# Quantum-Chemistry-Group-BNU/PyNQS

Measured on AMD Instinct MI355X. Metric: local energies/sec (whole node), higher is better.
Workload: dtype f64

## Files before the change

pynqs_amd/csrc/kernels_rbm_forward.hip:

```cpp
#include "detcore.h"
#include "launch.h"
#include "rbm_math.h"

namespace pynqs {

constexpr int kHChunk = 8;

struct Prod {
  double re = 1.0, im = 0.0;
  double lin = 0.0, ang = 0.0;
  int e2 = 0;
  __device__ __forceinline__ void renorm() {
    int k;
    (void)frexp(fmax(fabs(re), fabs(im)), &k);
    re = ldexp(re, -k); im = ldexp(im, -k);
    e2 += k;
  }
  __device__ __forceinline__ bool finite() const { return fabs(re) < __builtin_inf() && fabs(im) < __builtin_inf(); }
  template <bool CPLX>
  __device__ __forceinline__ void times_2cosh(double x, double y) {
    const double ax = fabs(x);
    const double rho = exp(-2.0 * ax);
    lin += ax;
    if constexpr (CPLX) {
      const double sy = x < 0.0 ? -y : y;
      double sn, cs;
      sincos_mod(-2.0 * sy, sn, cs);
      const double u = fma(rho, cs, 1.0), v = rho * sn;
      const double nr = re * u - im * v;
      im = fma(re, v, im * u);
      re = nr;
      ang += sy;
    } else {
      re *= 1.0 + rho;
    }
  }
};

template <int FLAVOUR>
__device__ __forceinline__ void write_psi(double *__restrict__ psi, int64_t i, const Prod &P, double axr, double axi) {
  const double kLn2 = 0.693147180559945309417;
  if constexpr (FLAVOUR == PYNQS_RBM_REAL) {
    psi[i] = P.re * exp(axr + P.lin + kLn2 * (double)P.e2);
  } else if constexpr (FLAVOUR == PYNQS_RBM_TANH) {
    psi[i] = tanh(axr) * P.re * exp(P.lin + kLn2 * (double)P.e2);
  } else if constexpr (FLAVOUR == PYNQS_RBM_PHASE) {
    double sn, cs;
    sincos(axr + P.lin + log(P.re) + kLn2 * (double)P.e2, &sn, &cs);
    psi[2 * i] = cs; psi[2 * i + 1] = sn;
  } else {
    const double m = exp(axr + P.lin + kLn2 * (double)P.e2);
    double sn, cs;
    sincos(axi + P.ang, &sn, &cs);
    psi[2 * i] = m * (P.re * cs - P.im * sn);
    psi[2 * i + 1] = m * (P.re * sn + P.im * cs);
  }
}

template <int LEN, int FLAVOUR>
__device__ __forceinline__ void rbm_forward_row(const uint64_t (&ket)[LEN], int sorb, int H, const double *__restrict__ W,
                                                const double *__restrict__ hb, const double *__restrict__ vb, Prod &P, double &axr, double &axi) {
  constexpr bool CPLX = FLAVOUR == PYNQS_RBM_COMPLEX;
  for (int h0 = 0; h0 < H; h0 += kHChunk) {
    double tr[kHChunk], ti[kHChunk];
#pragma unroll
    for (int j = 0; j < kHChunk; ++j) {
      const int h = min(h0 + j, H - 1);
      tr[j] = CPLX ? hb[2 * h] : hb[h];
      ti[j] = CPLX ? hb[2 * h + 1] : 0.0;
    }
    for (int o = 0; o < sorb; ++o) {
      const double x = pm1_of<LEN>(ket, o);
#pragma unroll
      for (int j = 0; j < kHChunk; ++j) {
        const int h = min(h0 + j, H - 1);
        if constexpr (CPLX) {
          tr[j] = fma(x, W[((size_t)h * sorb + o) * 2], tr[j]);
          ti[j] = fma(x, W[((size_t)h * sorb + o) * 2 + 1], ti[j]);
        } else {
          tr[j] = fma(x, W[(size_t)h * sorb + o], tr[j]);
        }
      }
    }
#pragma unroll
    for (int j = 0; j < kHChunk; ++j)
      if (h0 + j < H) P.template times_2cosh<CPLX>(tr[j], ti[j]);
    P.renorm();
  }
  axr = 0.0; axi = 0.0;
  if (vb) {
    for (int o = 0; o < sorb; ++o) {
      const double x = pm1_of<LEN>(ket, o);
      if constexpr (CPLX) { axr = fma(x, vb[2 * o], axr); axi = fma(x, vb[2 * o + 1], axi); }
      else axr = fma(x, vb[o], axr);
    }
  }
}

template <int LEN, int FLAVOUR>
__global__ __launch_bounds__(kBlock) void rbm_forward_kernel(const uint64_t *__restrict__ onv, int64_t n, int sorb, int H,
                                                             const double *__restrict__ W, const double *__restrict__ hb,
                                                             const double *__restrict__ vb, double *__restrict__ psi) {
  const int64_t i = (int64_t)blockIdx.x * kBlock + threadIdx.x;
  const int64_t row = i < n ? i : n - 1;
  uint64_t ket[LEN];
#pragma unroll
  for (int w = 0; w < LEN; ++w) ket[w] = onv[row * LEN + w];
  Prod P;
  double axr, axi;
  rbm_forward_row<LEN, FLAVOUR>(ket, sorb, H, W, hb, vb, P, axr, axi);
  if (i >= n) return;
  write_psi<FLAVOUR>(psi, i, P, axr, axi);
}

__host__ __device__ inline int children_hp(int H) { return (H + 2) | 1; }

template <bool CPLX>
__global__ __launch_bounds__(kBlock) void rbm_children_factors_kernel(int sorb, int H, const double *__restrict__ W, const double *__restrict__ vb,
                                                                      double *__restrict__ factors) {
  constexpr int C = CPLX ? 2 : 1;
  const int HP = children_hp(H);
  const int idx = blockIdx.x * kBlock + threadIdx.x;
  if (idx == 0) factors[(size_t)(2 * sorb + 1) * HP * C] = 0.0;
  if (idx >= (2 * sorb + 1) * HP) return;
  const int row = idx / HP, h = idx - row * HP, o = row >> 1;
  const double sign = (row & 1) ? -1.0 : 1.0;
  double re = 0.0, im = 0.0;
  if (row == 2 * sorb) {
    re = h < H ? 1.0 : 0.0;
  } else if (h < H) {
    const double wr = W[((size_t)h * sorb + o) * C], wi = CPLX ? W[((size_t)h * sorb + o) * C + 1] : 0.0;
    const double m = fabs(4.0 * wr) <= 80.0 ? exp(-4.0 * sign * wr) : __builtin_nan("");
    if constexpr (CPLX) {
      double sn, cs;
      sincos(-4.0 * sign * wi, &sn, &cs);
      re = m * cs; im = m * sn;
    } else {
      re = m;
    }
  } else if (h == H) {
#pragma unroll 16
    for (int k = 0; k < H; ++k) {
      re += W[((size_t)k * sorb + o) * C];
      if constexpr (CPLX) im += W[((size_t)k * sorb + o) * C + 1];
    }
    re *= 2.0 * sign; im *= 2.0 * sign;
  } else if (h == H + 1 && vb) {
    re = 2.0 * sign * vb[(size_t)o * C];
    if constexpr (CPLX) im = 2.0 * sign * vb[(size_t)o * C + 1];
  }
  factors[(size_t)idx * C] = re;
  if constexpr (CPLX) factors[(size_t)idx * C + 1] = im;
}

constexpr int kParentChunk = 4;

template <int LEN, bool CPLX>
__global__ __launch_bounds__(kBlock) void rbm_children_parents_kernel(const uint64_t *__restrict__ onv, int64_t n, int sorb, int H,
                                                                      const double *__restrict__ W, const double *__restrict__ hb,
                                                                      const double *__restrict__ vb, const double *__restrict__ factors,
                                                                      double *__restrict__ table) {
  constexpr int C = CPLX ? 2 : 1;
  const int64_t i = (int64_t)blockIdx.x * kBlock + threadIdx.x;
  const int64_t row = i < n ? i : n - 1;
  const int h0 = (int)blockIdx.y * kParentChunk;
  uint64_t ket[LEN];
#pragma unroll
  for (int w = 0; w < LEN; ++w) ket[w] = onv[row * LEN + w];
  double *__restrict__ out = table + (size_t)row * (size_t)(H + 2) * C;
  double tr[kParentChunk], ti[kParentChunk];
#pragma unroll
  for (int j = 0; j < kParentChunk; ++j) {
    const int h = min(h0 + j, H - 1);
    tr[j] = CPLX ? hb[2 * h] : hb[h];
    ti[j] = CPLX ? hb[2 * h + 1] : 0.0;
  }
  for (int o = 0; o < sorb; ++o) {
    const double x = pm1_of<LEN>(ket, o);
#pragma unroll
    for (int j = 0; j < kParentChunk; ++j) {
      const int h = min(h0 + j, H - 1);
      tr[j] = fma(x, W[((size_t)h * sorb + o) * C], tr[j]);
      if constexpr (CPLX) ti[j] = fma(x, W[((size_t)h * sorb + o) * C + 1], ti[j]);
    }
  }
#pragma unroll
  for (int j = 0; j < kParentChunk; ++j) {
    if (h0 + j < H && i < n) {
      if (!(tr[j] > -340.0)) const_cast<double *>(factors)[(size_t)(2 * sorb + 1) * children_hp(H) * C] = 1.0;
      const double m = exp(-2.0 * tr[j]);
      if constexpr (CPLX) {
        double sn, cs;
        sincos_mod(-2.0 * ti[j], sn, cs);
        out[(size_t)(h0 + j) * 2] = m * cs;
        out[(size_t)(h0 + j) * 2 + 1] = m * sn;
      } else {
        out[h0 + j] = m;
      }
    }
  }
  if (blockIdx.y != 0) return;
  const int HP = children_hp(H);
  double sr = 0.0, si = 0.0, axr = 0.0, axi = 0.0;
  for (int h = 0; h < H; ++h) {
    sr += hb[(size_t)h * C];
    if constexpr (CPLX) si += hb[(size_t)h * C + 1];
  }
  for (int o = 0; o < sorb; ++o) {
    const double x = pm1_of<LEN>(ket, o);
    const double *__restrict__ f = factors + ((size_t)(2 * o) * HP + H) * C;
    sr = fma(0.5 * x, f[0], sr);
    axr = fma(0.5 * x, f[C], axr);
    if constexpr (CPLX) { si = fma(0.5 * x, f[1], si); axi = fma(0.5 * x, f[C + 1], axi); }
  }
  if (i >= n) return;
  out[(size_t)H * C] = sr;
  out[(size_t)(H + 1) * C] = axr;
  if constexpr (CPLX) { out[(size_t)H * C + 1] = si; out[(size_t)(H + 1) * C + 1] = axi; }
}

#ifndef PYNQS_CHILD_BLOCK
#define PYNQS_CHILD_BLOCK 1024
#endif
constexpr int kChildBlock = PYNQS_CHILD_BLOCK;

template <int LEN, int FLAVOUR>
__global__ __launch_bounds__(kChildBlock) void rbm_forward_children_kernel(const uint64_t *__restrict__ onv, int64_t n, const int32_t *__restrict__ count_dev,
                                                                      const int32_t *__restrict__ parent, const uint64_t *__restrict__ walkers,
                                                                      int64_t nwalkers, const double *__restrict__ table,
                                                                      const double *__restrict__ factors, int sorb, int H,
                                                                      const double *__restrict__ W, const double *__restrict__ hb,
                                                                      const double *__restrict__ vb, double *__restrict__ psi) {
  constexpr bool CPLX = FLAVOUR == PYNQS_RBM_COMPLEX;
  constexpr int C = CPLX ? 2 : 1;
  extern __shared__ __attribute__((aligned(16))) double wl[];
  const int HP = children_hp(H);
  int64_t cnt = n;
  if (count_dev) cnt = min((int64_t)max(*count_dev, 0), n);
  if (factors[(size_t)(2 * sorb + 1) * HP * C] != 0.0) {
    const int64_t rounds = (cnt + (int64_t)gridDim.x * kChildBlock - 1) / ((int64_t)gridDim.x * kChildBlock);
    for (int64_t r = 0; r < rounds; ++r) {
      const int64_t i = ((int64_t)r * gridDim.x + blockIdx.x) * kChildBlock + threadIdx.x;
      const int64_t row = i < cnt ? i : cnt - 1;
      uint64_t ket[LEN];
#pragma unroll
      for (int w = 0; w < LEN; ++w) ket[w] = onv[row * LEN + w];
      Prod P;
      double axr, axi;
      rbm_forward_row<LEN, FLAVOUR>(ket, sorb, H, W, hb, vb, P, axr, axi);
      if (i < cnt) write_psi<FLAVOUR>(psi, i, P, axr, axi);
    }
    return;
  }
  for (int idx = threadIdx.x; idx < (2 * sorb + 1) * HP * C; idx += kChildBlock) wl[idx] = factors[idx];
  __syncthreads();
  for (int64_t i = (int64_t)blockIdx.x * kChildBlock + threadIdx.x; i < cnt; i += (int64_t)gridDim.x * kChildBlock) {
    int64_t p = parent[i];
    bool stranger = p < 0 || p >= nwalkers;
    p = stranger ? 0 : p;
    int at[4];
#pragma unroll
    for (int q = 0; q < 4; ++q) at[q] = 2 * sorb * HP;
    int k = 0, nflip = 0;
#pragma unroll
    for (int w = 0; w < LEN; ++w) {
      const uint64_t xc = onv[i * LEN + w];
      uint64_t d = xc ^ walkers[p * LEN + w];
      nflip += __popcll(d);
#pragma unroll
      for (int t = 0; t < 4; ++t) {
        if (d && k < 4) {
          const int b = __builtin_ctzll(d);
          d &= d - 1;
          const int r = (2 * (64 * w + b) + (((xc >> b) & 1ull) ? 0 : 1)) * HP;
#pragma unroll
          for (int q = 0; q < 4; ++q)
            if (q == k) at[q] = r;
          ++k;
        }
      }
    }
    const double *__restrict__ tp = table + (size_t)p * (size_t)(H + 2) * C;
    Prod P;
    for (int h0 = 0; h0 < H; h0 += kHChunk) {
#pragma unroll
      for (int j = 0; j < kHChunk; ++j) {
        const int h = h0 + j;
        if (h < H) {
          double qr = tp[(size_t)h * C], qi = CPLX ? tp[(size_t)h * C + 1] : 0.0;
#pragma unroll
          for (int q = 0; q < 4; ++q) {
            const double fr = wl[(size_t)(at[q] + h) * C];
            if constexpr (CPLX) {
              const double fi = wl[(size_t)(at[q] + h) * C + 1];
              const double nr = qr * fr - qi * fi;
              qi = fma(qr, fi, qi * fr);
              qr = nr;
            } else {
              qr *= fr;
            }
          }
          if constexpr (CPLX) {
            const double u = 1.0 + qr;
            const double nr = P.re * u - P.im * qi;
            P.im = fma(P.re, qi, P.im * u);
            P.re = nr;
          } else {
            P.re *= 1.0 + qr;
          }
        }
      }
      P.renorm();
    }
    double axr = tp[(size_t)(H + 1) * C], axi = CPLX ? tp[(size_t)(H + 1) * C + 1] : 0.0;
    P.lin = tp[(size_t)H * C];
    P.ang = CPLX ? tp[(size_t)H * C + 1] : 0.0;
#pragma unroll
    for (int q = 0; q < 4; ++q) {
      P.lin += wl[(size_t)(at[q] + H) * C];
      axr += wl[(size_t)(at[q] + H + 1) * C];
      if constexpr (CPLX) {
        P.ang += wl[(size_t)(at[q] + H) * C + 1];
        axi += wl[(size_t)(at[q] + H + 1) * C + 1];
      }
    }
    stranger = stranger || nflip > 4 || !P.finite();
    if (__ballot(stranger)) {
      uint64_t ket[LEN];
#pragma unroll
      for (int w = 0; w < LEN; ++w) ket[w] = onv[i * LEN + w];
      Prod P2;
      double a2r, a2i;
      rbm_forward_row<LEN, FLAVOUR>(ket, sorb, H, W, hb, vb, P2, a2r, a2i);
      if (stranger) { P = P2; axr = a2r; axi = a2i; }
    }
    write_psi<FLAVOUR>(psi, i, P, axr, axi);
  }
}

template <int LEN, int FLAVOUR>
__global__ __launch_bounds__(kBlock) void rbm_forward_children_wave_kernel(const uint64_t *__restrict__ onv, int64_t n, const int32_t *__restrict__ count_dev,
                                                                           const int32_t *__restrict__ parent, const uint64_t *__restrict__ walkers,
                                                                           int64_t nwalkers, const double *__restrict__ table,
                                                                           const double *__restrict__ factors, int sorb, int H,
                                                                           const double *__restrict__ W, const double *__restrict__ hb,
                                                                           const double *__restrict__ vb, double *__restrict__ psi) {
  constexpr bool CPLX = FLAVOUR == PYNQS_RBM_COMPLEX;
  constexpr int C = CPLX ? 2 : 1;
  const int HP = children_hp(H);
  int64_t cnt = n;
  if (count_dev) cnt = min((int64_t)max(*count_dev, 0), n);
  if (factors[(size_t)(2 * sorb + 1) * HP * C] != 0.0) {
    const int64_t rounds = (cnt + (int64_t)gridDim.x * kBlock - 1) / ((int64_t)gridDim.x * kBlock);
    for (int64_t r = 0; r < rounds; ++r) {
      const int64_t i = ((int64_t)r * gridDim.x + blockIdx.x) * kBlock + threadIdx.x;
      const int64_t row = i < cnt ? i : cnt - 1;
      uint64_t ket[LEN];
#pragma unroll
      for (int w = 0; w < LEN; ++w) ket[w] = onv[row * LEN + w];
      Prod P;
      double axr, axi;
      rbm_forward_row<LEN, FLAVOUR>(ket, sorb, H, W, hb, vb, P, axr, axi);
      if (i < cnt) write_psi<FLAVOUR>(psi, i, P, axr, axi);
    }
    return;
  }
  const int lane = threadIdx.x & 63;
  const int wave = __builtin_amdgcn_readfirstlane((int)(threadIdx.x >> 6));
  const int64_t nwaves = (int64_t)gridDim.x * (kBlock / 64);
  constexpr int kWaveRows = 16;
  for (int64_t i0 = ((int64_t)blockIdx.x * (kBlock / 64) + wave) * kWaveRows; i0 < cnt; i0 += nwaves * kWaveRows)
  for (int64_t i = i0; i < min(i0 + kWaveRows, cnt); ++i) {
    int64_t p = parent[i];
    bool stranger = p < 0 || p >= nwalkers;
    p = stranger ? 0 : p;
    int at[4];
#pragma unroll
    for (int q = 0; q < 4; ++q) at[q] = 2 * sorb * HP;
    int k = 0, nflip = 0;
#pragma unroll
    for (int w = 0; w < LEN; ++w) {
      const uint64_t xc = onv[i * LEN + w];
      uint64_t d = xc ^ walkers[p * LEN + w];
      nflip += __popcll(d);
#pragma unroll
      for (int t = 0; t < 4; ++t) {
        if (d && k < 4) {
          const int b = __builtin_ctzll(d);
          d &= d - 1;
          const int r = (2 * (64 * w + b) + (((xc >> b) & 1ull) ? 0 : 1)) * HP;
#pragma unroll
          for (int q = 0; q < 4; ++q)
            if (q == k) at[q] = r;
          ++k;
        }
      }
    }
    const auto from_scratch = [&]() {
      uint64_t ket[LEN];
#pragma unroll
      for (int w = 0; w < LEN; ++w) ket[w] = onv[i * LEN + w];
      Prod P2;
      double a2r, a2i;
      rbm_forward_row<LEN, FLAVOUR>(ket, sorb, H, W, hb, vb, P2, a2r, a2i);
      if (lane == 0) write_psi<FLAVOUR>(psi, i, P2, a2r, a2i);
    };
    if (stranger || nflip > 4) {
      from_scratch();
      continue;
    }
    const double *__restrict__ tp = table + (size_t)p * (size_t)(H + 2) * C;
    Prod P;
    for (int h = lane; h < H; h += 64) {
      double qr = tp[(size_t)h * C], qi = CPLX ? tp[(size_t)h * C + 1] : 0.0;
#pragma unroll
      for (int q = 0; q < 4; ++q) {
        const double fr = factors[(size_t)(at[q] + h) * C];
        if constexpr (CPLX) {
          const double fi = factors[(size_t)(at[q] + h) * C + 1];
          const double nr = qr * fr - qi * fi;
          qi = fma(qr, fi, qi * fr);
          qr = nr;
        } else {
          qr *= fr;
        }
      }
      if constexpr (CPLX) {
        const double u = 1.0 + qr;
        const double nr = P.re * u - P.im * qi;
        P.im = fma(P.re, qi, P.im * u);
        P.re = nr;
      } else {
        P.re *= 1.0 + qr;
      }
      P.renorm();
    }
#pragma unroll
    for (int d = 32; d > 0; d >>= 1) {
      const double orr = __shfl_xor(P.re, d), oi = CPLX ? __shfl_xor(P.im, d) : 0.0;
      const int oe = __shfl_xor(P.e2, d);
      if constexpr (CPLX) {
        const double nr = P.re * orr - P.im * oi;
        P.im = fma(P.re, oi, P.im * orr);
        P.re = nr;
      } else {
        P.re *= orr;
      }
      P.e2 += oe;
    }
    P.renorm();
    if (__ballot(!P.finite())) {
      from_scratch();
      continue;
    }
    if (lane == 0) {
      double axr = tp[(size_t)(H + 1) * C], axi = CPLX ? tp[(size_t)(H + 1) * C + 1] : 0.0;
      P.lin = tp[(size_t)H * C];
      P.ang = CPLX ? tp[(size_t)H * C + 1] : 0.0;
#pragma unroll
      for (int q = 0; q < 4; ++q) {
        P.lin += factors[(size_t)(at[q] + H) * C];
        axr += factors[(size_t)(at[q] + H + 1) * C];
        if constexpr (CPLX) {
          P.ang += factors[(size_t)(at[q] + H) * C + 1];
          axi += factors[(size_t)(at[q] + H + 1) * C + 1];
        }
      }
      write_psi<FLAVOUR>(psi, i, P, axr, axi);
    }
  }
}

}

using namespace pynqs;

extern "C" int pynqs_rbm_forward(const uint64_t *onv, int64_t n, int sorb, const double *weights, const double *hidden_bias,
                                 const double *visible_bias, int nhidden, int flavour, double *psi, void *stream) {
  pynqs::DeviceScope device_scope_(onv);
  if (n < 0 || n > 0x7fffffffll * kBlock || sorb < 1 || sorb > kMaxSorb || nhidden < 1) return set_error(PYNQS_EINVAL, "bad n/sorb/nhidden");
  if (flavour != PYNQS_RBM_REAL && flavour != PYNQS_RBM_TANH && flavour != PYNQS_RBM_PHASE && flavour != PYNQS_RBM_COMPLEX)
    return set_error(PYNQS_EINVAL, "bad flavour");
  if (n == 0) return PYNQS_OK;
  if (!onv || !weights || !hidden_bias || !psi) return set_error(PYNQS_EINVAL, "null pointer");
  const int len = (sorb - 1) / 64 + 1;
  const uint32_t grid = (uint32_t)((n + kBlock - 1) / kBlock);
  hipStream_t st = (hipStream_t)stream;
#define PYNQS_RF(F) hipLaunchKernelGGL((rbm_forward_kernel<LEN, F>), dim3(grid), dim3(kBlock), 0, st, onv, n, sorb, nhidden, weights, hidden_bias, visible_bias, psi)
  DISPATCH_LEN(len, {
    switch (flavour) {
      case PYNQS_RBM_REAL: PYNQS_RF(PYNQS_RBM_REAL); break;
      case PYNQS_RBM_TANH: PYNQS_RF(PYNQS_RBM_TANH); break;
      case PYNQS_RBM_PHASE: PYNQS_RF(PYNQS_RBM_PHASE); break;
      default: PYNQS_RF(PYNQS_RBM_COMPLEX); break;
    }
  });
#undef PYNQS_RF
  return check_launch("rbm_forward");
}

static size_t children_lds_bytes(int sorb, int nhidden, int flavour) {
  return (size_t)(2 * sorb + 1) * (size_t)children_hp(nhidden) * (flavour == PYNQS_RBM_COMPLEX ? 16 : 8);
}

static bool children_flavour_ok(int flavour) {
  return flavour == PYNQS_RBM_REAL || flavour == PYNQS_RBM_TANH || flavour == PYNQS_RBM_PHASE || flavour == PYNQS_RBM_COMPLEX;
}

extern "C" int pynqs_rbm_forward_children_supported(int sorb, int nhidden, int flavour) {
  if (sorb < 1 || sorb > kMaxSorb || nhidden < 1 || !children_flavour_ok(flavour)) return 0;
  return 1;
}
static bool children_table_in_lds(int sorb, int nhidden, int flavour) {
  static const int force = getenv("PYNQS_RBM_CHILDREN_WAVE") ? atoi(getenv("PYNQS_RBM_CHILDREN_WAVE")) : -1;
  return force != 1 && children_lds_bytes(sorb, nhidden, flavour) <= 64 * 1024;
}

extern "C" int64_t pynqs_rbm_children_table_bytes(int64_t nwalkers, int sorb, int nhidden, int flavour) {
  if (nwalkers < 0 || sorb < 1 || sorb > kMaxSorb || nhidden < 1 || !children_flavour_ok(flavour)) return -1;
  const int64_t c = flavour == PYNQS_RBM_COMPLEX ? 16 : 8;
  return nwalkers * (nhidden + 2) * c + (int64_t)children_lds_bytes(sorb, nhidden, flavour) + 8;
}

extern "C" int pynqs_rbm_children_prepare(const uint64_t *walkers, int64_t nwalkers, int sorb, const double *weights, const double *hidden_bias,
                                          const double *visible_bias, int nhidden, int flavour, void *table, void *stream) {
  pynqs::DeviceScope device_scope_(table);
  if (nwalkers < 0 || nwalkers > 0x7fffffffll * kBlock || sorb < 1 || sorb > kMaxSorb || nhidden < 1 || !children_flavour_ok(flavour))
    return set_error(PYNQS_EINVAL, "bad nwalkers/sorb/nhidden/flavour");
  if (!weights || !hidden_bias || !table || (nwalkers > 0 && !walkers)) return set_error(PYNQS_EINVAL, "null pointer");
  const bool cplx = flavour == PYNQS_RBM_COMPLEX;
  const int len = (sorb - 1) / 64 + 1;
  hipStream_t st = (hipStream_t)stream;
  double *parents = (double *)table;
  double *factors = parents + (size_t)nwalkers * (size_t)(nhidden + 2) * (cplx ? 2 : 1);
  const uint32_t gf = (uint32_t)(((2 * sorb + 1) * children_hp(nhidden) + kBlock - 1) / kBlock);
  if (cplx) hipLaunchKernelGGL((rbm_children_factors_kernel<true>), dim3(gf), dim3(kBlock), 0, st, sorb, nhidden, weights, visible_bias, factors);
  else hipLaunchKernelGGL((rbm_children_factors_kernel<false>), dim3(gf), dim3(kBlock), 0, st, sorb, nhidden, weights, visible_bias, factors);
  if (nwalkers > 0) {
    const dim3 grid((uint32_t)((nwalkers + kBlock - 1) / kBlock), (uint32_t)((nhidden + kParentChunk - 1) / kParentChunk));
    if (grid.y > 65535u) return set_error(PYNQS_EINVAL, "too many hidden units");
    DISPATCH_LEN(len, {
      if (cplx)
        hipLaunchKernelGGL((rbm_children_parents_kernel<LEN, true>), grid, dim3(kBlock), 0, st, walkers, nwalkers, sorb, nhidden, weights,
                           hidden_bias, visible_bias, factors, parents);
      else
        hipLaunchKernelGGL((rbm_children_parents_kernel<LEN, false>), grid, dim3(kBlock), 0, st, walkers, nwalkers, sorb, nhidden, weights,
                           hidden_bias, visible_bias, factors, parents);
    });
  }
  return check_launch("rbm_children_prepare");
}

extern "C" int pynqs_rbm_forward_children(const uint64_t *onv, int64_t n, const int32_t *count_dev, const int32_t *parent,
                                          const uint64_t *walkers, int64_t nwalkers, const void *table, int sorb, const double *weights,
                                          const double *hidden_bias, const double *visible_bias, int nhidden, int flavour, double *psi,
                                          void *stream) {
  pynqs::DeviceScope device_scope_(onv);
  if (n < 0 || n > 0x7fffffffll * kBlock || nwalkers < 0 || sorb < 1 || sorb > kMaxSorb || nhidden < 1) return set_error(PYNQS_EINVAL, "bad n/sorb/nhidden");
  if (!pynqs_rbm_forward_children_supported(sorb, nhidden, flavour))
    return set_error(PYNQS_EINVAL, "rbm_forward_children: bad flavour");
  if (n == 0) return PYNQS_OK;
  if (!onv || !parent || !walkers || !table || !psi || !weights || !hidden_bias || nwalkers == 0) return set_error(PYNQS_EINVAL, "null pointer");
  const int len = (sorb - 1) / 64 + 1;
  int64_t blocks = (n + kChildBlock - 1) / kChildBlock;
  if (blocks > 1024) blocks = 1024;
  const uint32_t grid = (uint32_t)blocks;
  const size_t lds = children_lds_bytes(sorb, nhidden, flavour);
  const double *parents = (const double *)table;
  const double *factors = parents + (size_t)nwalkers * (size_t)(nhidden + 2) * (flavour == PYNQS_RBM_COMPLEX ? 2 : 1);
  hipStream_t st = (hipStream_t)stream;
  const bool in_lds = children_table_in_lds(sorb, nhidden, flavour);
  int64_t wblocks = (n + (kBlock / 64) * 16 - 1) / ((kBlock / 64) * 16);
  if (wblocks > 256 * 32) wblocks = 256 * 32;
#define PYNQS_RC(F)                                                                                                                          \
  do {                                                                                                                                       \
    if (in_lds)                                                                                                                              \
      hipLaunchKernelGGL((rbm_forward_children_kernel<LEN, F>), dim3(grid), dim3(kChildBlock), lds, st, onv, n, count_dev, parent, walkers,  \
                         nwalkers, parents, factors, sorb, nhidden, weights, hidden_bias, visible_bias, psi);                                \
    else                                                                                                                                     \
      hipLaunchKernelGGL((rbm_forward_children_wave_kernel<LEN, F>), dim3((uint32_t)wblocks), dim3(kBlock), 0, st, onv, n, count_dev,        \
                         parent, walkers, nwalkers, parents, factors, sorb, nhidden, weights, hidden_bias, visible_bias, psi);               \
  } while (0)
  DISPATCH_LEN(len, {
    switch (flavour) {
      case PYNQS_RBM_REAL: PYNQS_RC(PYNQS_RBM_REAL); break;
      case PYNQS_RBM_TANH: PYNQS_RC(PYNQS_RBM_TANH); break;
      case PYNQS_RBM_PHASE: PYNQS_RC(PYNQS_RBM_PHASE); break;
      default: PYNQS_RC(PYNQS_RBM_COMPLEX); break;
    }
  });
#undef PYNQS_RC
  return check_launch("rbm_forward_children");
}
```

pynqs_amd/csrc/kernels_reduce_onepass.hip:

```cpp
#include "detcore.h"
#include "launch.h"
#include "plan.h"
#include "plan_dev.h"
#include "plan_tiles.h"
#include "reduce_common.h"
#include "reduce_list.h"

namespace pynqs {




template <int LEN, typename T, bool SAMPLED>
struct KeepSink {
  T eps;
  uint32_t chunk, nchunks, tS;
  int64_t seg_base;
  volatile uint32_t *run;
  WinnerList wl;
  uint32_t *bufc;
  T *bufh;
  volatile uint32_t *dstat;
  double *tsum;
  uint32_t *kept_total;
// ... 303 lines not shown
__global__ __launch_bounds__(kBlock) void reduce_onepass_kernel(const uint64_t *__restrict__ bra, SDParams p, PlanLayout pl, uint32_t nchunks,
                                                                uint32_t chunk_len, uint32_t max_tiles, const T *__restrict__ plan, T eps,
                                                                uint32_t nsample, uint64_t seed, uint32_t wl_cap, OnepassOut<T> o) {
  extern __shared__ __attribute__((aligned(16))) unsigned char smem[];
  __shared__ uint32_t next_tile, kept_total, wl_n;
  __shared__ int32_t wl_base;
  __shared__ uint32_t wave_run[kBlock / 64];
  __shared__ double s_part[kBlock / 64 + 1];
  __shared__ uint32_t s_parti[kBlock / 64 + 1];
  uint64_t walker;
  uint32_t chunk;
  map_workgroup(nchunks, false, walker, chunk);
  o.parent = (int32_t)walker;
  const uint64_t slot = walker * nchunks + chunk;
  const int tid = threadIdx.x, lane = tid & 63, wave = tid >> 6;
  const int64_t seg_base = (int64_t)slot * ((int64_t)o.fixed + o.cap_d);
  if (tid == 0) { next_tile = 0; kept_total = 0; wl_n = 0; }
  unsigned char *extra = smem + ((lds_bytes(p, sizeof(T)) + 15) & ~(size_t)15);
  volatile uint32_t *dstat = reinterpret_cast<volatile uint32_t *>(extra);
  extra += ((size_t)max_tiles * 4 + 15) & ~(size_t)15;
  double *tsum = reinterpret_cast<double *>(extra);
  uint32_t *dinfo = reinterpret_cast<uint32_t *>(extra + (SAMPLED ? (size_t)max_tiles * 8 : 0));
  WinnerList wl;
  wl.n = &wl_n;
  wl.cap = wl_cap;
  wl.slot = reinterpret_cast<uint32_t *>(smem + onepass_lds(p, sizeof(T), max_tiles, SAMPLED, 0));
  wl.col = wl.slot + wl_cap;
  for (uint32_t i = tid; i < max_tiles; i += kBlock) {
    dstat[i] = 0u;
    if constexpr (SAMPLED) { tsum[i] = 0.0; dinfo[i] = 0u; }
  }
  for (uint32_t i = tid; i < o.fixed; i += kBlock) o.rec_col[seg_base + i] = -1;
  if constexpr (SAMPLED) {
    for (uint32_t i = tid; i < nsample; i += kBlock) o.srec_col[(int64_t)walker * nsample + i] = -1;
  }
  Walker<LEN> wk;
  load_walker<LEN>(bra + walker * LEN, wk);
  const LdsLayout L = carve_lds(smem, p);
  const int nocc = build_walker_tables<LEN>(wk, p, L);

  const uint32_t tS_all = (p.d1 + kSinglesPerTile - 1) / kSinglesPerTile;
  const uint32_t tS = tS_all > chunk ? (tS_all - chunk + nchunks - 1) / nchunks : 0;
  T *quarter = reinterpret_cast<T *>(L.scratch) + wave * (kDiagTile / 4);
  {
    KeepSink<LEN, T, SAMPLED> sink;
    sink.eps = eps; sink.chunk = chunk; sink.nchunks = nchunks; sink.tS = tS; sink.seg_base = seg_base;
    sink.run = wave_run + wave; sink.wl = wl;
    sink.bufh = quarter;
    sink.bufc = reinterpret_cast<uint32_t *>(quarter + kOneTileCols);
    sink.dstat = dstat; sink.tsum = tsum; sink.kept_total = &kept_total;
    sink.p = &p; sink.L = &L; sink.wk = &wk; sink.o = o; sink.tile = 0xffffffffu; sink.sub = 0.0;
    visit_tiles<LEN, T>(p, pl, L, nocc, plan, wk, nchunks, chunk, chunk_len, 0u, &next_tile, sink);
    sink.flush();
  }
  flush_winner_list<LEN, T>(o, wl, &wl_base, p, L, wk);
  if (tid == 0) {
    o.seg_count[slot] = (int32_t)kept_total;
    if (kept_total > o.cap_d) {
      atomicOr(reinterpret_cast<unsigned int *>(o.counters + 1), 1u);
      atomicMax(o.counters + 2, (int32_t)kept_total);
    }
  }
  if constexpr (SAMPLED) {
    const uint32_t per = (max_tiles + kBlock - 1) / kBlock;
    const uint32_t b0 = min((uint32_t)tid * per, max_tiles), b1 = min(b0 + per, max_tiles);
    double local = 0.0;
    for (uint32_t i = b0; i < b1; ++i) local += tsum[i];
    double incl = op_scan(local, lane);
    if (lane == 63) s_part[wave] = incl;
    __syncthreads();
    double before = 0.0, total = 0.0;
    for (int w = 0; w < kBlock / 64; ++w) {
      if (w < wave) before += s_part[w];
      total += s_part[w];
    }
    double run = before + incl - local;
    for (uint32_t i = b0; i < b1; ++i) { run += tsum[i]; tsum[i] = run; }
    __syncthreads();
    const double Srow = total;
    if (tid == 0 && o.row_sum) o.row_sum[walker] = Srow;
    const uint64_t key = op_mix64((o.seed_dev ? seed + *o.seed_dev : seed) ^ op_mix64(slot));
    if (Srow > 0.0) {
      for (uint32_t k = tid; k < nsample; k += kBlock) {
        const uint64_t r = op_mix64(key ^ op_mix64(0xffffffff00000000ull | k));
        const double target = (double)(r >> 11) * 0x1.0p-53 * Srow;
        uint32_t lo = 0, hi = max_tiles;
        while (lo < hi) {
          const uint32_t mid = (lo + hi) >> 1;
          if (tsum[mid] > target) hi = mid; else lo = mid + 1;
        }
        if (lo >= max_tiles) lo = max_tiles - 1;
        while (lo > 0 && !(tsum[lo] > tsum[lo - 1])) --lo;
        atomicAdd(&dinfo[lo], 1u);
      }
    }
    __syncthreads();
    uint32_t lsum = 0;
    for (uint32_t i = b0; i < b1; ++i) lsum += dinfo[i];
    uint32_t iscan = lsum;
#pragma unroll
    for (int d = 1; d < 64; d <<= 1) {
      const uint32_t ov = __shfl_up(iscan, d);
      if (lane >= d) iscan += ov;
    }
    if (lane == 63) s_parti[wave] = iscan;
    __syncthreads();
    uint32_t ibefore = 0;
    for (int w = 0; w < wave; ++w) ibefore += s_parti[w];
    uint32_t off = ibefore + iscan - lsum;
    for (uint32_t i = b0; i < b1; ++i) {
      const uint32_t c = dinfo[i];
      dinfo[i] = (off << 16) | c;
      off += c;
    }
    if (tid == 0) next_tile = 0;
    __syncthreads();
    unsigned char *mine = reinterpret_cast<unsigned char *>(dinfo) + (((size_t)max_tiles * 4 + 15) & ~(size_t)15) + (size_t)wave * kDrawLdsPerWave;
    DrawLds S;
    S.prefix = reinterpret_cast<double *>(mine);
    S.run = reinterpret_cast<volatile double *>(mine + (size_t)kOneTileCols * 8);
    S.cs = reinterpret_cast<uint32_t *>(mine + (size_t)kOneTileCols * 8 + 8);
    S.hits = S.cs + kOneTileCols;
    S.ncols = reinterpret_cast<volatile uint32_t *>(S.hits + kOneTileCols);
    DrawSink<LEN, T> sink{eps, S, &p, &L, &wk, dinfo, Srow / (double)nsample, key, (int64_t)walker * nsample, o, wl, 0xffffffffu};
    visit_tiles<LEN, T>(p, pl, L, nocc, plan, wk, nchunks, chunk, chunk_len, 0u, &next_tile, sink);
    sink.flush();
    flush_winner_list<LEN, T>(o, wl, &wl_base, p, L, wk);
  }
}


template <int LEN, typename T, bool SAMPLED, bool CACHED = false>
__global__ __launch_bounds__(kBlock) __attribute__((amdgpu_waves_per_eu(8, 8)))
void reduce_onepass_list_kernel(const uint64_t *__restrict__ bra, SDParams p, PlanLayout pl, uint32_t nchunks, uint32_t chunk_len, uint32_t max_tiles,
                                const T *__restrict__ plan, T eps, uint32_t nsample, uint64_t seed, uint32_t P, OnepassOut<T> o) {
  static_assert(CACHED || !SAMPLED, "the re-enumerating form has its own kernel");
  reduce_onepass_list_body<LEN, T, SAMPLED, CACHED>(bra, p, pl, nchunks, chunk_len, max_tiles, plan, eps, nsample, seed, P, o);
}

template <int LEN, typename T, bool SAMPLED = false, bool GTILE = false>
__global__ __launch_bounds__(kBlock) void reduce_onepass_list_flush_kernel(const uint64_t *__restrict__ bra, SDParams p, PlanLayout pl, uint32_t nchunks,
                                                                           uint32_t chunk_len, uint32_t max_tiles, const T *__restrict__ plan, T eps,
                                                                           uint32_t nsample, uint64_t seed, uint32_t P, OnepassOut<T> o) {
  reduce_onepass_list_body<LEN, T, SAMPLED, false, true, GTILE>(bra, p, pl, nchunks, chunk_len, max_tiles, plan, eps, nsample, seed, P, o);
}

template <int LEN, typename T, bool GTILE = false>
__global__ __launch_bounds__(kBlock) void reduce_onepass_list_redraw_kernel(const uint64_t *__restrict__ bra, SDParams p, PlanLayout pl, uint32_t nchunks,
                                                                            uint32_t chunk_len, uint32_t max_tiles, const T *__restrict__ plan, T eps,
                                                                            uint32_t nsample, uint64_t seed, uint32_t P, OnepassOut<T> o) {
  reduce_onepass_list_body<LEN, T, true, false, false, GTILE>(bra, p, pl, nchunks, chunk_len, max_tiles, plan, eps, nsample, seed, P, o);
}

template <typename T, bool CPLX>
__global__ __launch_bounds__(kBlock) void reduce_contract_kernel(int64_t nbatch, uint32_t nchunks, uint32_t fixed, uint32_t cap_d,
                                                                 uint32_t nsample, const int32_t *__restrict__ rec_col,
                                                                 const T *__restrict__ rec_w, const int32_t *__restrict__ rec_link,
                                                                 const int32_t *__restrict__ seg_count, const int32_t *__restrict__ srec_col,
                                                                 const T *__restrict__ srec_w, const int32_t *__restrict__ srec_link,
                                                                 const int32_t *__restrict__ dedup_i32, int slot_i32, int row_off, uint32_t ucap,
                                                                 const double *__restrict__ psi_u, const double *__restrict__ psi_t, int divide,
                                                                 double *__restrict__ eloc, double *__restrict__ psi_x) {
  const int lane = threadIdx.x & 63;
  const int64_t walker = (int64_t)blockIdx.x * (kBlock / 64) + (threadIdx.x >> 6);
  if (walker >= nbatch) return;
  double ar = 0.0, ai = 0.0, xr = 0.0, xi = 0.0;
  bool bad = false;
  auto amp = [&](int32_t link, double &re, double &im) {
    const double *src;
    int64_t at;
    if (link >= kDirectLink) {
      src = psi_u; at = link - kDirectLink;
      if ((uint32_t)at >= ucap) { bad = true; re = im = 0.0; return; }
    } else if (link >= 0) {
      if (!dedup_i32) { bad = true; re = im = 0.0; return; }
      const int32_t row = dedup_i32[(int64_t)link * slot_i32 + row_off];
      if (row < 0 || (uint32_t)row >= ucap) { bad = true; re = im = 0.0; return; }
      src = psi_u; at = row;
    } else if (link <= -2) {
      src = psi_t; at = -2 - (int64_t)link;
    } else { bad = true; re = im = 0.0; return; }
    if constexpr (CPLX) { re = src[2 * at]; im = src[2 * at + 1]; }
    else { re = src[at]; im = 0.0; }
  };
  auto visit = [&](int32_t col, double w, int32_t link) {
    if (col < 0) return;
    double re, im;
    amp(link, re, im);
    ar += w * re; ai += w * im;
    if (col == 0) { xr = re; xi = im; }
  };
  const int64_t stride = (int64_t)fixed + cap_d;
  for (uint32_t c = 0; c < nchunks; ++c) {
    const int64_t seg = walker * nchunks + c, base = seg * stride;
    const uint32_t kept = (uint32_t)seg_count[seg];
    if (kept > cap_d) bad = true;
    const uint32_t nslots = fixed + min(kept, cap_d);
    for (uint32_t i = lane; i < nslots; i += 64) visit(rec_col[base + i], (double)rec_w[base + i], rec_link[base + i]);
  }
  for (uint32_t i = lane; i < nsample; i += 64) {
    const int64_t at = walker * nsample + i;
    visit(srec_col[at], (double)srec_w[at], srec_link[at]);
  }
#pragma unroll
  for (int d = 32; d > 0; d >>= 1) {
    ar += __shfl_xor(ar, d); ai += __shfl_xor(ai, d);
    xr += __shfl_xor(xr, d); xi += __shfl_xor(xi, d);
  }
  const bool anybad = __ballot(bad) != 0;
  if (lane == 0) {
    if (anybad) { ar = ai = __builtin_nan(""); }
    if constexpr (CPLX) {
      if (divide) scaled_cdiv(ar, ai, xr, xi, ar, ai);
      eloc[2 * walker] = ar;
      eloc[2 * walker + 1] = ai;
      psi_x[2 * walker] = xr; psi_x[2 * walker + 1] = xi;
    } else {
      eloc[walker] = divide ? ar / xr : ar;
      psi_x[walker] = xr;
    }
  }
}

}

using namespace pynqs;

static int onepass_geometry(int64_t nbatch, const SDParams &p, bool sampled, uint32_t *nchunks, uint32_t *chunk_len, uint32_t *max_tiles,
                            uint32_t *fixed) {
  const uint32_t ncomb = p.nsd + 1;
  if (sampled) {
    *nchunks = 1;
    *chunk_len = (ncomb + 255u) & ~255u;
  } else {
    plan_chunks(nbatch, ncomb, nchunks, chunk_len);
  }
  *max_tiles = max_tiles_per_chunk(p, *nchunks, *chunk_len);
  const uint32_t tS_all = (p.d1 + kSinglesPerTile - 1) / kSinglesPerTile;
  *fixed = kFixedHead + ((tS_all + *nchunks - 1) / *nchunks) * kSinglesPerTile;
  return 0;
}

static size_t onepass_static_lds(int) { return 16 + (kBlock / 64) * 4 + (kBlock / 64 + 1) * 12 + 64; }

extern "C" int pynqs_reduce_onepass_geometry(int64_t nbatch, int sorb, int nele, int noA, int noB, int eps_sample, int64_t *out4) {
  SDParams p;
  PlanLayout pl;
  if (!out4) return set_error(PYNQS_EINVAL, "null pointer");
  if (!make_sd_params(sorb, nele, noA, noB, &p) || !make_plan_layout(sorb, &pl)) return set_error(PYNQS_EINVAL, "bad sorb/noA/noB (even sorb in [2, 192])");
  if (nbatch < 0 || nbatch > 0x7fffffffll || eps_sample < 0 || eps_sample > 65535) return set_error(PYNQS_EINVAL, "bad nbatch / eps_sample (at most 65535 draws)");
  uint32_t nchunks, chunk_len, max_tiles, fixed;
  onepass_geometry(nbatch, p, eps_sample > 0, &nchunks, &chunk_len, &max_tiles, &fixed);
  const int len = (sorb - 1) / 64 + 1;
  const int64_t slots = out4[2];
  out4[0] = nbatch * (int64_t)nchunks;
  out4[1] = fixed;
  out4[2] = slots > 0 ? slots * dedup_slot_words(len) * 8 : 0;
  const bool lookback = onepass_lds(p, 8, max_tiles, eps_sample > 0, winner_list_cap(eps_sample)) + onepass_static_lds(len) <= 160 * 1024;
  const bool flushing = eps_sample > 0 && p.nsd + 1 > 65536 &&
                        onepass_list_lds(p, 8, max_tiles, true, 2048, (uint32_t)eps_sample, false, true) + 256 + onepass_static_lds(len) <= 160 * 1024;
  out4[3] = lookback || flushing ? 1 : 0;
  return PYNQS_OK;
}

constexpr uint32_t kLongRow = 65536;
struct OnepassForm {
  uint32_t P;
  bool use_list, use_cache, use_flush, use_gtile;
  size_t lds;
  bool use_split = false;
  bool use_row32 = false;
};
static OnepassForm onepass_form(const SDParams &p, size_t esz, uint32_t max_tiles, uint32_t fixed, uint64_t cap_doubles, int eps_sample,
                                bool have_cache, uint32_t chunk_len, bool no_table, bool have_tile_scratch = false, bool have_row_f32 = false) {
  static const int list_env = getenv("PYNQS_OP_LIST") ? atoi(getenv("PYNQS_OP_LIST")) : -1;
  static const int cache_env = getenv("PYNQS_OP_CACHE") ? atoi(getenv("PYNQS_OP_CACHE")) : -1;
  static const int flush_env = getenv("PYNQS_OP_FLUSH") ? atoi(getenv("PYNQS_OP_FLUSH")) : -1;
  const bool sampled = eps_sample > 0;
  const uint64_t seg_cap = (uint64_t)fixed + cap_doubles;
  OnepassForm f;
  f.P = 64;
  while (f.P < seg_cap && f.P < (1u << 20)) f.P <<= 1;
  const bool want_cache = sampled && have_cache && cache_env != 0;
  const bool gtile = sampled && !want_cache && have_tile_scratch;
  const size_t lds_list = onepass_list_lds(p, esz, max_tiles, sampled, f.P, (uint32_t)eps_sample, want_cache, gtile);
  const bool list_fits = seg_cap <= 2048 && lds_list + 256 <= 160 * 1024;
  f.use_list = list_env == 0 ? false : (list_fits && (list_env == 1 || seg_cap <= 1024 || p.nsd + 1 > kLongRow));
  f.use_cache = want_cache && f.use_list;
  f.use_gtile = gtile && f.use_list;
  f.lds = f.use_list ? lds_list : onepass_lds(p, esz, max_tiles, sampled, winner_list_cap(eps_sample));
  static const int split_env = getenv("PYNQS_OP_SPLIT") ? atoi(getenv("PYNQS_OP_SPLIT")) : -1;
  if (sampled && have_row_f32 && split_env != 0 && list_env != 0 && seg_cap <= 1024 && reduce_draw_supported(p, eps_sample)) {
    const uint32_t slots = ((uint32_t)seg_cap + 1u) & ~1u;
    const size_t lds_a = onepass_list_lds(p, esz, max_tiles, true, slots, (uint32_t)eps_sample, false, false, true);
    if (lds_a + 256 <= 160 * 1024) {
      f.P = slots;
      f.use_list = true; f.use_split = true; f.use_cache = f.use_gtile = f.use_flush = false; f.lds = lds_a;
      return f;
    }
  }
  const bool gtile_f = sampled && have_tile_scratch;
  const uint32_t flush_P = flush_list_slots((p.sorb - 1) / 64 + 1, sampled);
  const size_t lds_flush = onepass_list_lds(p, esz, max_tiles, sampled, flush_P, (uint32_t)eps_sample, false, gtile_f);
  const bool long_row = p.nsd + 1 > kLongRow;
  f.use_flush = !f.use_list && flush_env != 0 && lds_flush + 256 <= 160 * 1024 &&
                (long_row || flush_env == 1 || no_table || cap_doubles * 10 <= (uint64_t)chunk_len);
  if (f.use_flush) { f.use_gtile = gtile_f; f.use_cache = false; }
  if (f.use_flush) { f.P = flush_P; f.lds = lds_flush; }
  static const int row32_env = getenv("PYNQS_OP_ROW32") ? atoi(getenv("PYNQS_OP_ROW32")) : -1;
  const bool from_list = f.use_list && !f.use_cache && flush_env != 0;
  if ((f.use_flush || from_list) && sampled && have_row_f32 && row32_env != 0 && row32_fits(esz, flush_P, (uint32_t)eps_sample, gtile_f)) {
    const size_t lds_r = onepass_list_lds(p, esz, max_tiles, true, flush_P, (uint32_t)eps_sample, false, gtile_f, false, true);
    const size_t wg_old = (size_t)160 * 1024 / ((f.use_flush ? lds_flush : f.lds) + 512), wg_new = (size_t)160 * 1024 / (lds_r + 512);
    if (lds_r + 256 <= 160 * 1024 && (row32_env == 1 || wg_new > wg_old || (uint64_t)eps_sample * 8 >= max_tiles)) {
      f.use_row32 = true; f.use_flush = true; f.use_list = false; f.use_cache = false; f.use_gtile = gtile_f; f.P = flush_P; f.lds = lds_r;
    }
  }
  return f;
}

extern "C" int64_t pynqs_reduce_onepass_tile_scratch_bytes(int64_t nbatch, int sorb, int nele, int noA, int noB, int eps_sample) {
  SDParams p;
  PlanLayout pl;
  if (!make_sd_params(sorb, nele, noA, noB, &p) || !make_plan_layout(sorb, &pl) || nbatch < 0 || nbatch > 0x7fffffffll || eps_sample < 0 || eps_sample > 65535) {
    set_error(PYNQS_EINVAL, "bad arguments");
    return -1;
  }
  if (eps_sample == 0) return 0;
  uint32_t nchunks, chunk_len, max_tiles, fixed;
  onepass_geometry(nbatch, p, true, &nchunks, &chunk_len, &max_tiles, &fixed);
  return (int64_t)((size_t)nbatch * tile_scratch_stride(max_tiles));
}

extern "C" int pynqs_reduce_onepass_list_capacity(int64_t nbatch, int sorb, int nele, int noA, int noB, int dtype, int eps_sample,
                                                  int with_row_cache, int without_table, int64_t *cap_doubles) {
  SDParams p;
  PlanLayout pl;
  if (!cap_doubles) return set_error(PYNQS_EINVAL, "null pointer");
  if (!make_sd_params(sorb, nele, noA, noB, &p) || !make_plan_layout(sorb, &pl)) return set_error(PYNQS_EINVAL, "bad sorb/noA/noB (even sorb in [2, 192])");
  if (nbatch < 0 || nbatch > 0x7fffffffll || eps_sample < 0 || eps_sample > 65535 || (dtype != PYNQS_F32 && dtype != PYNQS_F64))
    return set_error(PYNQS_EINVAL, "bad nbatch / eps_sample / dtype");
  uint32_t nchunks, chunk_len, max_tiles, fixed;
  onepass_geometry(nbatch, p, eps_sample > 0, &nchunks, &chunk_len, &max_tiles, &fixed);
  const size_t esz = dtype == PYNQS_F64 ? 8 : 4;
  auto listed = [&](uint64_t cap) {
    const OnepassForm f = onepass_form(p, esz, max_tiles, fixed, cap, eps_sample, with_row_cache != 0, chunk_len, without_table != 0,
                                       eps_sample > 0 && with_row_cache == 0);
    return (f.use_list || f.use_flush) && f.lds + onepass_static_lds(0) <= 160 * 1024;
  };
  *cap_doubles = -1;
  if (listed((uint64_t)1 << 29)) { *cap_doubles = ((int64_t)1 << 30) - 1; return PYNQS_OK; }
  for (uint32_t seg = 2048; seg >= 128; seg >>= 1) {
    if (seg < fixed) break;
    if (listed(seg - fixed)) { *cap_doubles = (int64_t)(seg - fixed); break; }
  }
  if ((int64_t)(chunk_len / 10) > *cap_doubles && listed(chunk_len / 10)) *cap_doubles = chunk_len / 10;
// ... 135 lines not shown
```

Before: 9.601 million.

## Software-pipeline children RBM kernel and batch contract-kernel gathers with hot path

Restructures the children forward kernel. Parent-table values for the next hidden chunk are prefetched while the current chunk is processed, shared-memory factor reads are grouped between scheduling barriers, and the LDS fill is unrolled. The grid-stride loop becomes one row per thread with no grid cap, and blocks with no rows exit early. psi is written before the fallback, and the fallback pins its pointers to scalar registers. Separately, the contract kernel loads G slots per lane at once, splitting out a hot direct-link path and a wave-uniform cold path, to raise memory-level parallelism. The cost is more register pressure and possibly more blocks, each refilling LDS.

```diff
diff --git a/pynqs_amd/csrc/kernels_rbm_forward.hip b/pynqs_amd/csrc/kernels_rbm_forward.hip
--- a/pynqs_amd/csrc/kernels_rbm_forward.hip
+++ b/pynqs_amd/csrc/kernels_rbm_forward.hip
@@ -1,3 +1,5 @@
+#include <type_traits>
+
 #include "detcore.h"
 #include "launch.h"
 #include "rbm_math.h"
@@ -222,6 +224,11 @@
 #ifndef PYNQS_CHILD_BLOCK
 #define PYNQS_CHILD_BLOCK 1024
 #endif
+#ifndef PYNQS_CHILD_GROUP
+#define PYNQS_CHILD_GROUP 4
+#endif
+constexpr int kChildGroup = PYNQS_CHILD_GROUP;
+static_assert(kHChunk % kChildGroup == 0, "whole groups per chunk");
 constexpr int kChildBlock = PYNQS_CHILD_BLOCK;
 
 template <int LEN, int FLAVOUR>
@@ -252,9 +259,19 @@
     }
     return;
   }
-  for (int idx = threadIdx.x; idx < (2 * sorb + 1) * HP * C; idx += kChildBlock) wl[idx] = factors[idx];
+  if ((int64_t)blockIdx.x * kChildBlock >= cnt) return;
+  {
+    const int words = (2 * sorb + 1) * HP * C;
+    int idx = threadIdx.x;
+    for (; idx + 3 * kChildBlock < words; idx += 4 * kChildBlock) {
+      const double a = factors[idx], b = factors[idx + kChildBlock], c = factors[idx + 2 * kChildBlock], d = factors[idx + 3 * kChildBlock];
+      wl[idx] = a; wl[idx + kChildBlock] = b; wl[idx + 2 * kChildBlock] = c; wl[idx + 3 * kChildBlock] = d;
+    }
+    for (; idx < words; idx += kChildBlock) wl[idx] = factors[idx];
+  }
   __syncthreads();
-  for (int64_t i = (int64_t)blockIdx.x * kChildBlock + threadIdx.x; i < cnt; i += (int64_t)gridDim.x * kChildBlock) {
+  const int64_t i = (int64_t)blockIdx.x * kChildBlock + threadIdx.x;
+  if (i < cnt) {
     int64_t p = parent[i];
     bool stranger = p < 0 || p >= nwalkers;
     p = stranger ? 0 : p;
@@ -282,34 +299,67 @@
     }
     const double *__restrict__ tp = table + (size_t)p * (size_t)(H + 2) * C;
     Prod P;
-    for (int h0 = 0; h0 < H; h0 += kHChunk) {
-#pragma unroll
-      for (int j = 0; j < kHChunk; ++j) {
-        const int h = h0 + j;
-        if (h < H) {
-          double qr = tp[(size_t)h * C], qi = CPLX ? tp[(size_t)h * C + 1] : 0.0;
-#pragma unroll
-          for (int q = 0; q < 4; ++q) {
-            const double fr = wl[(size_t)(at[q] + h) * C];
-            if constexpr (CPLX) {
-              const double fi = wl[(size_t)(at[q] + h) * C + 1];
-              const double nr = qr * fr - qi * fi;
-              qi = fma(qr, fi, qi * fr);
-              qr = nr;
-            } else {
-              qr *= fr;
-            }
-          }
-          if constexpr (CPLX) {
-            const double u = 1.0 + qr;
-            const double nr = P.re * u - P.im * qi;
-            P.im = fma(P.re, qi, P.im * u);
-            P.re = nr;
-          } else {
-            P.re *= 1.0 + qr;
-          }
+    struct Factors { double re[4], im[4]; };
+    const auto read_factors = [&](int h) {
+      Factors f;
+#pragma unroll
+      for (int q = 0; q < 4; ++q) {
+        f.re[q] = wl[(size_t)(at[q] + h) * C];
+        f.im[q] = CPLX ? wl[(size_t)(at[q] + h) * C + 1] : 0.0;
+      }
+      return f;
+    };
+    const auto unit = [&](double qr, double qi, const Factors &f) {
+#pragma unroll
+      for (int q = 0; q < 4; ++q) {
+        if constexpr (CPLX) {
+          const double nr = qr * f.re[q] - qi * f.im[q];
+          qi = fma(qr, f.im[q], qi * f.re[q]);
+          qr = nr;
+        } else {
+          qr *= f.re[q];
         }
       }
+      if constexpr (CPLX) {
+        const double u = 1.0 + qr;
+        const double nr = P.re * u - P.im * qi;
+        P.im = fma(P.re, qi, P.im * u);
+        P.re = nr;
+      } else {
+        P.re *= 1.0 + qr;
+      }
+    };
+    double qr[kHChunk], qi[kHChunk];
+    const auto load_q = [&](int j, int h) {
+      h = min(h, H - 1);
+      qr[j] = tp[(size_t)h * C]; qi[j] = CPLX ? tp[(size_t)h * C + 1] : 0.0;
+    };
+#pragma unroll
+    for (int j = 0; j < kHChunk; ++j) load_q(j, j);
+    const auto chunk = [&](int h0, auto ahead) {
+#pragma unroll
+      for (int j0 = 0; j0 < kHChunk; j0 += kChildGroup) {
+        Factors f[kChildGroup];
+#pragma unroll
+        for (int j = 0; j < kChildGroup; ++j) f[j] = read_factors(h0 + j0 + j);
+        __builtin_amdgcn_sched_barrier(0);
+#pragma unroll
+        for (int j = 0; j < kChildGroup; ++j) {
+          unit(qr[j0 + j], qi[j0 + j], f[j]);
+          if constexpr (decltype(ahead)::value) load_q(j0 + j, h0 + kHChunk + j0 + j);
+        }
+        __builtin_amdgcn_sched_barrier(0);
+      }
+      P.renorm();
+    };
+    int h0 = 0;
+    for (; h0 + kHChunk < H; h0 += kHChunk) chunk(h0, std::true_type{});
+    if (h0 + kHChunk == H) {
+      chunk(h0, std::false_type{});
+    } else {
+#pragma unroll
+      for (int j = 0; j < kHChunk - 1; ++j)
+        if (h0 + j < H) unit(qr[j], qi[j], read_factors(h0 + j));
       P.renorm();
     }
     double axr = tp[(size_t)(H + 1) * C], axi = CPLX ? tp[(size_t)(H + 1) * C + 1] : 0.0;
@@ -325,16 +375,18 @@
       }
     }
     stranger = stranger || nflip > 4 || !P.finite();
+    write_psi<FLAVOUR>(psi, i, P, axr, axi);
     if (__ballot(stranger)) {
       uint64_t ket[LEN];
 #pragma unroll
       for (int w = 0; w < LEN; ++w) ket[w] = onv[i * LEN + w];
       Prod P2;
       double a2r, a2i;
-      rbm_forward_row<LEN, FLAVOUR>(ket, sorb, H, W, hb, vb, P2, a2r, a2i);
-      if (stranger) { P = P2; axr = a2r; axi = a2i; }
-    }
-    write_psi<FLAVOUR>(psi, i, P, axr, axi);
+      const double *W2 = W, *hb2 = hb, *vb2 = vb;
+      asm volatile("" : "+s"(W2), "+s"(hb2), "+s"(vb2));
+      rbm_forward_row<LEN, FLAVOUR>(ket, sorb, H, W2, hb2, vb2, P2, a2r, a2i);
+      if (stranger) write_psi<FLAVOUR>(psi, i, P2, a2r, a2i);
+    }
   }
 }
 
@@ -562,9 +614,7 @@
   if (n == 0) return PYNQS_OK;
   if (!onv || !parent || !walkers || !table || !psi || !weights || !hidden_bias || nwalkers == 0) return set_error(PYNQS_EINVAL, "null pointer");
   const int len = (sorb - 1) / 64 + 1;
-  int64_t blocks = (n + kChildBlock - 1) / kChildBlock;
-  if (blocks > 1024) blocks = 1024;
-  const uint32_t grid = (uint32_t)blocks;
+  const uint32_t grid = (uint32_t)((n + kChildBlock - 1) / kChildBlock);
   const size_t lds = children_lds_bytes(sorb, nhidden, flavour);
   const double *parents = (const double *)table;
   const double *factors = parents + (size_t)nwalkers * (size_t)(nhidden + 2) * (flavour == PYNQS_RBM_COMPLEX ? 2 : 1);
diff --git a/pynqs_amd/csrc/kernels_reduce_onepass.hip b/pynqs_amd/csrc/kernels_reduce_onepass.hip
--- a/pynqs_amd/csrc/kernels_reduce_onepass.hip
+++ b/pynqs_amd/csrc/kernels_reduce_onepass.hip
@@ -479,6 +479,11 @@
   reduce_onepass_list_body<LEN, T, true, false, false, GTILE>(bra, p, pl, nchunks, chunk_len, max_tiles, plan, eps, nsample, seed, P, o);
 }
 
+#ifndef PYNQS_CONTRACT_GROUPS
+#define PYNQS_CONTRACT_GROUPS 4
+#endif
+constexpr int kContractGroups = PYNQS_CONTRACT_GROUPS;
+
 template <typename T, bool CPLX>
 __global__ __launch_bounds__(kBlock) void reduce_contract_kernel(int64_t nbatch, uint32_t nchunks, uint32_t fixed, uint32_t cap_d,
                                                                  uint32_t nsample, const int32_t *__restrict__ rec_col,
@@ -488,47 +493,76 @@
                                                                  const int32_t *__restrict__ dedup_i32, int slot_i32, int row_off, uint32_t ucap,
                                                                  const double *__restrict__ psi_u, const double *__restrict__ psi_t, int divide,
                                                                  double *__restrict__ eloc, double *__restrict__ psi_x) {
+  constexpr int G = kContractGroups;
   const int lane = threadIdx.x & 63;
   const int64_t walker = (int64_t)blockIdx.x * (kBlock / 64) + (threadIdx.x >> 6);
   if (walker >= nbatch) return;
   double ar = 0.0, ai = 0.0, xr = 0.0, xi = 0.0;
   bool bad = false;
-  auto amp = [&](int32_t link, double &re, double &im) {
+  auto amp_cold = [&](int32_t link, double &re, double &im) {
     const double *src;
     int64_t at;
-    if (link >= kDirectLink) {
-      src = psi_u; at = link - kDirectLink;
-      if ((uint32_t)at >= ucap) { bad = true; re = im = 0.0; return; }
-    } else if (link >= 0) {
-      if (!dedup_i32) { bad = true; re = im = 0.0; return; }
+    if (link >= 0) {
+      if (!dedup_i32) { bad = true; return; }
       const int32_t row = dedup_i32[(int64_t)link * slot_i32 + row_off];
-      if (row < 0 || (uint32_t)row >= ucap) { bad = true; re = im = 0.0; return; }
+      if (row < 0 || (uint32_t)row >= ucap) { bad = true; return; }
       src = psi_u; at = row;
     } else if (link <= -2) {
       src = psi_t; at = -2 - (int64_t)link;
-    } else { bad = true; re = im = 0.0; return; }
+    } else { bad = true; return; }
     if constexpr (CPLX) { re = src[2 * at]; im = src[2 * at + 1]; }
-    else { re = src[at]; im = 0.0; }
+    else { re = src[at]; }
   };
-  auto visit = [&](int32_t col, double w, int32_t link) {
-    if (col < 0) return;
-    double re, im;
-    amp(link, re, im);
-    ar += w * re; ai += w * im;
-    if (col == 0) { xr = re; xi = im; }
+  auto visit = [&](const int32_t *__restrict__ colp, const T *__restrict__ wp, const int32_t *__restrict__ linkp, uint32_t n) {
+    for (uint32_t i0 = 0; i0 < n; i0 += 64 * G) {
+      int32_t col[G], link[G];
+      double w[G], re[G], im[G];
+#pragma unroll
+      for (int g = 0; g < G; ++g) {
+        const uint32_t i = i0 + 64 * g + lane;
+        col[g] = -1; link[g] = -1; w[g] = 0.0;
+        if (i < n) { col[g] = colp[i]; w[g] = (double)wp[i]; link[g] = linkp[i]; }
+      }
+      bool cold = false;
+#pragma unroll
+      for (int g = 0; g < G; ++g) {
+        re[g] = 0.0; im[g] = 0.0;
+        if (col[g] >= 0) {
+          if (link[g] >= kDirectLink) {
+            const uint32_t at = (uint32_t)(link[g] - kDirectLink);
+            if (at < ucap) {
+              if constexpr (CPLX) { re[g] = psi_u[2 * (size_t)at]; im[g] = psi_u[2 * (size_t)at + 1]; }
+              else re[g] = psi_u[at];
+            } else {
+              bad = true;
+            }
+          } else {
+            cold = true;
+          }
+        }
+      }
+      if (__ballot(cold)) {
+#pragma unroll
+        for (int g = 0; g < G; ++g)
+          if (col[g] >= 0 && link[g] < kDirectLink) amp_cold(link[g], re[g], im[g]);
+      }
+#pragma unroll
+      for (int g = 0; g < G; ++g) {
+        if (col[g] >= 0) {
+          ar += w[g] * re[g]; ai += w[g] * im[g];
+          if (col[g] == 0) { xr = re[g]; xi = im[g]; }
+        }
+      }
+    }
   };
   const int64_t stride = (int64_t)fixed + cap_d;
   for (uint32_t c = 0; c < nchunks; ++c) {
     const int64_t seg = walker * nchunks + c, base = seg * stride;
     const uint32_t kept = (uint32_t)seg_count[seg];
     if (kept > cap_d) bad = true;
-    const uint32_t nslots = fixed + min(kept, cap_d);
-    for (uint32_t i = lane; i < nslots; i += 64) visit(rec_col[base + i], (double)rec_w[base + i], rec_link[base + i]);
-  }
-  for (uint32_t i = lane; i < nsample; i += 64) {
-    const int64_t at = walker * nsample + i;
-    visit(srec_col[at], (double)srec_w[at], srec_link[at]);
-  }
+    visit(rec_col + base, rec_w + base, rec_link + base, fixed + min(kept, cap_d));
+  }
+  if (nsample) visit(srec_col + walker * nsample, srec_w + walker * nsample, srec_link + walker * nsample, nsample);
 #pragma unroll
   for (int d = 32; d > 0; d >>= 1) {
     ar += __shfl_xor(ar, d); ai += __shfl_xor(ai, d);
```

After: 9.722 million (median of 6 runs). 1.01x the previous value.
